# google-research/frame-interpolation

Measured on NVIDIA H100. Metric: interpolated_frames_per_sec_1080p, higher is better.
Workload: dtype f16x2-split (activations/weights as fp16 hi+lo planes; fp32 accumulate)

## Files before the change

### frame_interpolation_b200/csrc/film_conv3x3_tc.cu

```cuda
#include <cuda.h>
#include <cuda_runtime.h>
#include <stdint.h>

#include <type_traits>

#include "film_conv.h"
#include "film_tc_ptx.cuh"

namespace film {
namespace {
using namespace tc;

constexpr int kConsumers = 256;
constexpr int kThreads = kConsumers + 128;
__host__ __device__ constexpr int a_plane_bytes(int kc, int th, int tw) { return (th + 2) * tw * kc * 2; }
__host__ __device__ constexpr int a_stage_bytes(int kc, int th, int tw) { return 2 * a_plane_bytes(kc, th, tw); }
constexpr int kHaloW = 10;
__host__ __device__ constexpr int halo_box_bytes(int kc, int th) { return (th + 2) * kHaloW * kc * 2; }
__host__ __device__ constexpr int halo_plane_bytes(int kc, int th) { return (halo_box_bytes(kc, th) + 1023) & ~1023; }
__host__ __device__ constexpr int a_stage_bytes_h(int kc, int th, int tw, int halo, int planes = 2) {
  return planes * (halo ? halo_plane_bytes(kc, th) : a_plane_bytes(kc, th, tw));
}
constexpr int kMaxRing = 8;
constexpr int kSmemLimit = 227 * 1024;
constexpr int kBarBytes = 8 * (4 * kMaxRing + 4);
constexpr int kFixedBytes = kBarBytes + 16 + 512 * 4  + 64  + 1024  + 64;
constexpr int kHeadW3 = 64 * 32 * 4, kHeadMisc = 512;
constexpr int kHeadBytes = kHeadW3 + kHeadMisc;
constexpr int kPxnStageWg = 64 * 64 * 2;
constexpr int kPxnStageBytes = 2 * kPxnStageWg;
inline int epi_scratch_bytes(int epi_mode, int pxn) { return epi_mode == 3 ? kHeadBytes : pxn ? kPxnStageBytes : 0; }

__host__ __device__ inline int w_tap_bytes(int bn, int kc, int planes = 2) { return bn * kc * 2 * planes; }

template <int BN, int KC, bool kPartial, bool kHalo, bool kOne, bool kRes, bool kPxN = false>
__global__ void __launch_bounds__(kThreads, 1) k_conv3x3_tc(const ConvProblem* __restrict__ prob) {
  static_assert(!kPxN || (BN == 64 && KC == 64), "pixels on N: Cout = 64 (one M = 64 weight tile), 64-channel chunks");
  extern __shared__ uint8_t smem_raw[];
  constexpr bool one = kOne;
  const int planes = one ? 1 : 2;
  constexpr int kWPlane = BN * KC * 2;
  const int kWTap = kWPlane * planes;
  const int kTileH = prob->tile_h, kTileW = prob->tile_w;
  constexpr int kHaloTileH = kPxN ? 32 : 16;
  constexpr int kHaloBox = halo_box_bytes(KC, kHaloTileH), kHaloPlane = halo_plane_bytes(KC, kHaloTileH);
  constexpr bool halo = kHalo;
  const int kAPlane = halo ? kHaloPlane : a_plane_bytes(KC, kTileH, kTileW);
  const int kAStage = planes * kAPlane;
  const int kRowStep = kTileW * KC * 2;
  constexpr bool kFused = BN <= 128 && !kPxN;
  constexpr int kAccRegs = kPxN ? 64 : (kFused ? 2 * BN : BN) / 2;
  constexpr int kWgPx = kPxN ? 128 : 64;

  const int NA = prob->v2_na, NW = prob->v2_nw;
  const bool resident = prob->v2_resident != 0;
  const int nsrc = prob->nsrc;
  const int tiles_x = prob->tiles_x, tiles_per_img = prob->tiles_y * prob->tiles_x;
  const int cout = prob->cout;
  const int n_nt = (cout + BN - 1) / BN;
  const int ntiles = prob->B * tiles_per_img * n_nt;
  constexpr int kStageTaps = kHalo ? 9 : 3;
  constexpr bool kPacked = kPartial && kPxN;
  const int part_lo = prob->v2_part_lo, part_hi = prob->v2_part_hi;
  int nab = 0;
  for (int s = 0; s < nsrc; ++s) nab += prob->src[s].nchunk * (kHalo ? 1 : 3);
  const int nkb = nab * kStageTaps - (kPacked ? (part_hi - part_lo) * (kStageTaps - kStageTaps / 3) : 0);

  const FastDiv div_nt(n_nt, ntiles), div_img(tiles_per_img, ntiles), div_tx(tiles_x, ntiles);
  const bool pair = prob->pair != 0;
  const int rank = pair ? (int)cluster_ctarank() : 0;
  const int nsp = prob->B * tiles_per_img;
  const int nwork = pair ? ((nsp + 1) / 2) * n_nt : ntiles;
  const int w_first = pair ? (int)blockIdx.x >> 1 : (int)blockIdx.x, w_step = pair ? (int)gridDim.x >> 1 : (int)gridDim.x;
  auto decode = [&](int work, int& sp, int& nti) {
    div_nt.divmod(work, sp, nti);
    if (pair) sp = 2 * sp + rank;
  };

  const uint32_t raw = smem_u32(smem_raw);
  const uint32_t base = (raw + 1023u) & ~1023u;
  uint8_t* gen_base = smem_raw + (base - raw);
  const uint32_t a_base = base;
  const uint32_t w_base = a_base + (uint32_t)NA * kAStage;
  const uint32_t w_bytes = resident ? (uint32_t)nkb * kWTap : (uint32_t)NW * kWTap;
  const uint32_t tail = w_base + w_bytes;
  const uint32_t tail_off = (uint32_t)NA * kAStage + w_bytes;
  float* bias_smem = reinterpret_cast<float*>(gen_base + tail_off + kBarBytes + 16);
  int* src_tab = reinterpret_cast<int*>(gen_base + tail_off + kBarBytes + 16 + 512 * 4);

  const int warp = threadIdx.x >> 5, lane = threadIdx.x & 31;

  if (warp == 8 && lane == 0) {
    for (int s = 0; s < kMaxRing; ++s) {
      mbar_init(tail + 8u * s, 1);
      mbar_init(tail + 8u * (kMaxRing + s), 2);
      mbar_init(tail + 8u * (2 * kMaxRing + s), 1);
      mbar_init(tail + 8u * (3 * kMaxRing + s), pair ? 4 : 2);
    }
    for (int s = 0; s < kMaxSrc; ++s) {
      src_tab[2 * s] = s < nsrc ? prob->src[s].nchunk : 0;
      src_tab[2 * s + 1] = s < nsrc ? prob->src[s].c_off : 0;
      src_tab[2 * kMaxSrc + s] = s < nsrc ? prob->src[s].bswap : 0;
    }
    asm volatile("fence.mbarrier_init.release.cluster;" ::: "memory");
  }
  if (warp < 8)
    for (int i = threadIdx.x; i < n_nt * BN; i += kConsumers) bias_smem[i] = (i < cout) ? prob->bias[i] : 0.f;
  __syncthreads();
  if (pair) cluster_sync_all();
  auto leave = [&]() {
    if (pair) cluster_sync_all();
  };

  if (warp >= 8) {
    regs_dec<40>();
    if (warp > 8) {
      leave();
      return;
    }
    const CUtensorMap* tm_w_hi = &prob->tm_w_hi;
    const CUtensorMap* tm_w_lo = &prob->tm_w_lo;
    if (resident && elect_one()) {
      mbar_expect_tx(tail + 8u * (2 * kMaxRing), (uint32_t)nkb * kWTap);
      for (int kb = 0; kb < nkb; ++kb) {
        tma_load_2d(w_base + kb * kWTap, tm_w_hi, tail + 8u * (2 * kMaxRing), kb * KC, 0);
        if (!one) tma_load_2d(w_base + kb * kWTap + kWPlane, tm_w_lo, tail + 8u * (2 * kMaxRing), kb * KC, 0);
      }
    }
    __syncwarp();
    RingPos ra, rw;
    for (int tile = w_first; tile < nwork; tile += w_step) {
      int sp, nti, b, rem, ty, tx;
      decode(tile, sp, nti);
      div_img.divmod(sp, b, rem);
      div_tx.divmod(rem, ty, tx);
      const int n0 = nti * BN, y0 = ty * kTileH, x0 = tx * kTileW;
      {
        const int nt = tile + w_step;
        int next_sp, nnt;
        decode(nt < nwork ? nt : 0, next_sp, nnt);
        if (nt < nwork && next_sp != sp && next_sp < nsp && elect_one()) {
          int nb, nrem, nty, ntx;
          div_img.divmod(next_sp, nb, nrem);
          div_tx.divmod(nrem, nty, ntx);
          const int ny0 = nty * kTileH, nx0 = ntx * kTileW;
          for (int s = 0; s < nsrc; ++s)
            for (int ch = 0; ch < src_tab[2 * s]; ++ch) {
              const int cc = src_tab[2 * s + 1] + ch * KC;
              tma_prefetch_4d(&prob->tm_a_hi[s], cc, nx0 - 1, ny0 - 1, nb);
              if (!one) tma_prefetch_4d(&prob->tm_a_lo[s], cc, nx0 - 1, ny0 - 1, nb);
              if (!halo) {
                tma_prefetch_4d(&prob->tm_a_hi[s], cc, nx0 + 1, ny0 - 1, nb);
                if (!one) tma_prefetch_4d(&prob->tm_a_lo[s], cc, nx0 + 1, ny0 - 1, nb);
              }
            }
        }
        __syncwarp();
      }
      int kb = 0, ab = 0;
      for (int s = 0; s < nsrc; ++s) {
        const int nchunk = src_tab[2 * s], c_off = src_tab[2 * s + 1];
        const int bs = src_tab[2 * kMaxSrc + s] ? prob->B - 1 - b : b;
        const CUtensorMap* tm_hi = &prob->tm_a_hi[s];
        const CUtensorMap* tm_lo = &prob->tm_a_lo[s];
        for (int ch = 0; ch < nchunk; ++ch) {
          const int nst = halo ? 1 : 3;
          for (int dx = 0; dx < nst; ++dx, ++ab) {
            const int st = ra.stage;
            mbar_wait(tail + 8u * (kMaxRing + st), ra.phase ^ 1u);
            if (elect_one()) {
              const uint32_t sa = a_base + st * kAStage, bar = tail + 8u * st;
              mbar_expect_tx(bar, halo ? (uint32_t)(planes * kHaloBox) : (uint32_t)kAStage);
              tma_load_4d(sa, tm_hi, bar, c_off + ch * KC, x0 + dx - 1, y0 - 1, bs);
              if (!one) tma_load_4d(sa + kAPlane, tm_lo, bar, c_off + ch * KC, x0 + dx - 1, y0 - 1, bs);
            }
            __syncwarp();
            ra.advance(NA);
            if (!resident) {
              const bool packed = kPacked && ab >= part_lo && ab < part_hi;
              const int nblk = packed ? kStageTaps / 3 : kStageTaps;
              for (int t = 0; t < nblk; ++t, ++kb) {
                const int ws = rw.stage;
                mbar_wait(tail + 8u * (3 * kMaxRing + ws), rw.phase ^ 1u);
                if (elect_one()) {
                  const uint32_t sw = w_base + ws * kWTap, bar = tail + 8u * (2 * kMaxRing + ws);
                  mbar_expect_tx(bar, kWTap);
                  if (pair) {
                    const uint32_t hoff = (uint32_t)(rank * (kWPlane / 2));
                    tma_load_2d_mc(sw + hoff, &prob->tm_w_hi_half, bar, kb * KC, n0 + rank * (BN / 2), 3);
                    if (!one) tma_load_2d_mc(sw + kWPlane + hoff, &prob->tm_w_lo_half, bar, kb * KC, n0 + rank * (BN / 2), 3);
                  } else {
                    tma_load_2d(sw, tm_w_hi, bar, kb * KC, n0);
                    if (!one) tma_load_2d(sw + kWPlane, tm_w_lo, bar, kb * KC, n0);
                  }
                }
                __syncwarp();
                rw.advance(NW);
              }
            }
          }
        }
      }
    }
    leave();
    return;
  }

  regs_inc<232>();
  const int wg = warp >> 2;
  const int q = lane & 3;
  const int H = prob->H, W = prob->W, out_H = prob->out_H, out_W = prob->out_W, out_C = prob->out_C;
  const int out_c_off = prob->out_c_off, act = prob->act;
  sp_t* const out_hi = prob->out_hi;
  sp_t* const out_lo = prob->out_lo;
  sp_t* const pool_hi = prob->pool_hi;
  sp_t* const pool_lo = prob->pool_lo;
  const int pool_C = prob->pool_C;
  const bool do_pool = pool_hi != nullptr;
  const bool lo_skip = prob->out_lo_skip != 0;
  const bool rgb = prob->epi_mode == 2;
  const float* const head_w = prob->head_w4;
  float* const rgb_out = prob->head_v;
  const int crop_y = prob->crop_y, crop_x = prob->crop_x, crop_h = prob->crop_h, crop_w = prob->crop_w;
  const int64_t crop_pitch = prob->crop_pitch;
  const bool fhead = prob->epi_mode == 3;
  constexpr int kHid = BN <= 64 ? BN / 2 : 1;
  float* const w3s = reinterpret_cast<float*>(reinterpret_cast<uint8_t*>(src_tab) + 64);
  float* const hmisc = w3s + kHeadW3 / 4;
  if (fhead) {
    if constexpr (BN <= 64) {
      for (int i = threadIdx.x; i < BN * kHid; i += kConsumers) w3s[i] = prob->head_w3[i];
      for (int i = threadIdx.x; i < kHid; i += kConsumers) hmisc[i] = prob->head_b3[i];
      for (int i = threadIdx.x; i < 2 * kHid; i += kConsumers) hmisc[kHid + i] = prob->head_w4[i];
      if (threadIdx.x < 2) hmisc[3 * kHid + threadIdx.x] = prob->head_b4[threadIdx.x];
    }
    asm volatile("bar.sync 1, %0;" ::"r"(kConsumers) : "memory");
  }
  const float* const head_vup = prob->head_vup;
  float* const head_res = prob->head_res;
  float* const head_vout = prob->head_v;

  if (resident) mbar_wait(tail + 8u * (2 * kMaxRing), 0);
  const bool is_leader = (threadIdx.x & 127) == 0;
  const uint32_t w_empty_peer = pair ? map_to_cta(tail + 8u * (3 * kMaxRing), (uint32_t)(rank ^ 1)) : 0u;
  auto release_w = [&](int slot) {
    mbar_arrive(tail + 8u * (3 * kMaxRing + slot));
    if (pair) mbar_arrive_cluster(w_empty_peer + 8u * slot);
  };
  {
    constexpr int kWTapC = kWPlane * (kOne ? 1 : 2);
    constexpr uint32_t kPx = KC * 2;
    const uint32_t a_row0 = kHalo ? (uint32_t)(wg * (kWgPx / 8) * kHaloW) * kPx : (uint32_t)(wg * kWgPx) * kPx;
    const uint32_t sbo = kHalo ? kHaloW * kPx : 8 * kPx;
    RingPos ra, rw;
    float acc[kAccRegs];
    for (int tile = w_first; tile < nwork; tile += w_step) {
      int kb = 0;
      int rel_a = -1, rel_w = -1;
      auto retire = [&](int next_a, int next_w) {
        wgmma_commit();
        wgmma_wait<1>();
        if (is_leader) {
          if (rel_a >= 0) mbar_arrive(tail + 8u * (kMaxRing + rel_a));
          if (rel_w >= 0) release_w(rel_w);
        }
        rel_a = next_a;
        rel_w = next_w;
      };
      auto stage = [&](auto ksteps_c, auto tpb_c) {
        constexpr int kSteps = decltype(ksteps_c)::value, kTpb = decltype(tpb_c)::value;
        constexpr int kBlocks = kStageTaps / kTpb;
        const int st = ra.stage;
        mbar_wait(tail + 8u * st, ra.phase);
        const uint32_t sa = a_base + st * kAStage + a_row0;
        const uint32_t lo_off = (uint32_t)(kHalo ? kHaloPlane : kAPlane);
        if constexpr (kRes) {
          const uint64_t a0 = make_desc_sbo<KC>(sa, sbo);
          const uint64_t lo_delta = (uint64_t)(lo_off >> 4);
          const uint64_t row_delta = (uint64_t)(kRowStep >> 4);
          const uint64_t w0 = make_desc_kc<KC>(w_base + kb * kWTapC);
          const uint32_t first = (kb == 0) ? 0u : 1u;
          wgmma_fence();
#pragma unroll
          for (int t = 0; t < kStageTaps; ++t) {
            const uint64_t a_hi = a0 + (kHalo ? (uint64_t)((((t % 3) * kHaloW + t / 3) * kPx) >> 4) : (uint64_t)t * row_delta);
            const uint64_t a_lo = a_hi + lo_delta;
            const uint64_t w_hi = w0 + (uint64_t)(((t / kTpb) * kWTapC + (t % kTpb) * kSteps * 32) >> 4);
            const uint64_t w_lo = w_hi + (uint64_t)(kWPlane >> 4);
#pragma unroll
            for (int k = 0; k < kSteps; ++k) {
              const uint64_t adv = (uint64_t)(k * 32 >> 4);
              const uint32_t accf = (t == 0 && k == 0) ? first : 1u;
              if constexpr (kPxN) {
                wgmma<128>(acc, w_hi + adv, a_hi + adv, accf);
                if constexpr (!kOne) {
                  wgmma<128>(acc, w_lo + adv, a_hi + adv, 1u);
                  wgmma<128>(acc, w_hi + adv, a_lo + adv, 1u);
                }
              } else if constexpr (kOne) {
                wgmma<BN>(acc, a_hi + adv, w_hi + adv, accf);
              } else if constexpr (kFused) {
                wgmma<BN>(acc, a_hi + adv, w_hi + adv, accf);
                wgmma<BN>(acc + BN / 2, a_hi + adv, w_lo + adv, accf);
                wgmma<BN>(acc, a_lo + adv, w_hi + adv, 1u);
              } else {
                wgmma<BN>(acc, a_lo + adv, w_hi + adv, accf);
                wgmma<BN>(acc, a_hi + adv, w_lo + adv, 1u);
                wgmma<BN>(acc, a_hi + adv, w_hi + adv, 1u);
              }
            }
          }
          retire(st, -1);
          kb += kBlocks;
        } else {
          for (int blk = 0; blk < kBlocks; ++blk, ++kb) {
            uint32_t sw;
            int ws = -1;
            if (resident) {
              sw = w_base + kb * kWTap;
            } else {
              ws = rw.stage;
              mbar_wait(tail + 8u * (2 * kMaxRing + ws), rw.phase);
              sw = w_base + ws * kWTap;
            }
            const uint32_t first = (kb == 0) ? 0u : 1u;
            wgmma_fence();
#pragma unroll
            for (int u = 0; u < kTpb; ++u) {
              const int t = blk * kTpb + u;
              const uint32_t off = kHalo ? (uint32_t)((t % 3) * kHaloW + t / 3) * kPx : (uint32_t)(t * kRowStep);
              const uint64_t a_hi = make_desc_sbo<KC>(sa + off, sbo);
              const uint64_t a_lo = make_desc_sbo<KC>(sa + lo_off + off, sbo);
              const uint64_t wk = (uint64_t)((u * kSteps * 32) >> 4);
              const uint64_t w_hi = make_desc_kc<KC>(sw) + wk, w_lo = make_desc_kc<KC>(sw + kWPlane) + wk;
#pragma unroll
              for (int k = 0; k < kSteps; ++k) {
                const uint64_t adv = (uint64_t)(k * 32 >> 4);
                const uint32_t accf = (u == 0 && k == 0) ? first : 1u;
                if constexpr (kPxN) {
                  wgmma<128>(acc, w_hi + adv, a_hi + adv, accf);
                  if constexpr (!kOne) {
                    wgmma<128>(acc, w_lo + adv, a_hi + adv, 1u);
                    wgmma<128>(acc, w_hi + adv, a_lo + adv, 1u);
                  }
                } else if constexpr (kOne) {
                  wgmma<BN>(acc, a_hi + adv, w_hi + adv, accf);
                } else if constexpr (kFused) {
                  wgmma<BN>(acc, a_hi + adv, w_hi + adv, accf);
                  wgmma<BN>(acc + BN / 2, a_hi + adv, w_lo + adv, accf);
                  wgmma<BN>(acc, a_lo + adv, w_hi + adv, 1u);
                } else {
                  wgmma<BN>(acc, a_lo + adv, w_hi + adv, accf);
                  wgmma<BN>(acc, a_hi + adv, w_lo + adv, 1u);
                  wgmma<BN>(acc, a_hi + adv, w_hi + adv, 1u);
                }
              }
            }
            retire(blk == kBlocks - 1 ? st : -1, ws);
            if (!resident) rw.advance(NW);
          }
        }
        ra.advance(NA);
      };
      using Full = std::integral_constant<int, KC / 16>;
      using One = std::integral_constant<int, 1>;
      if constexpr (kPartial) {
        for (int ab = 0; ab < part_lo; ++ab) stage(Full{}, One{});
        for (int ab = part_lo; ab < part_hi; ++ab) stage(One{}, std::integral_constant<int, kPacked ? 3 : 1>{});
        for (int ab = part_hi; ab < nab; ++ab) stage(Full{}, One{});
      } else {
        for (int ab = 0; ab < nab; ++ab) stage(Full{}, One{});
      }
      wgmma_wait<0>();
      if (is_leader) {
        if (rel_a >= 0) mbar_arrive(tail + 8u * (kMaxRing + rel_a));
        if (rel_w >= 0) release_w(rel_w);
      }
      acc_fence<kAccRegs>(acc);

      int sp, nti, b, rem, ty, tx;
      decode(tile, sp, nti);
      div_img.divmod(sp, b, rem);
      div_tx.divmod(rem, ty, tx);
      const int n0 = nti * BN;
      const bool live = sp < nsp;
      if constexpr (kPxN) {
        const int c0 = 16 * (warp & 3) + (lane >> 2);
        const float bias0 = bias_smem[c0], bias1 = bias_smem[c0 + 8];
#pragma unroll
        for (int i = 0; i < kAccRegs; ++i) {
          const float f = acc[i] + ((i & 2) ? bias1 : bias0);
          acc[i] = act ? leaky(f) : f;
        }
        const int y_wg = ty * kTileH + 16 * wg, x_t = tx * kTileW;
        if (do_pool) {
          const int px = x_t + 2 * q;
#pragma unroll
          for (int j = 0; j < 16; j += 2) {
            const int py = y_wg + j;
            const bool ok = live && (py >> 1) < (out_H >> 1) && (px >> 1) < (out_W >> 1) && !(lane & 4);
            const int64_t ppix = ((int64_t)b * (out_H >> 1) + (py >> 1)) * (out_W >> 1) + (px >> 1);
#pragma unroll
            for (int h = 0; h < 2; ++h) {
              const int i = 4 * j + 2 * h;
              const float v = ((acc[i] + acc[i + 1]) + (acc[i + 4] + acc[i + 5])) * 0.25f;
              const float vn = __shfl_xor_sync(0xffffffffu, v, 4);
              if (ok) {
                uint32_t hi, lo;
                split_pack2(v, vn, hi, lo);
                *reinterpret_cast<uint32_t*>(pool_hi + ppix * pool_C + c0 + 8 * h) = hi;
                *reinterpret_cast<uint32_t*>(pool_lo + ppix * pool_C + c0 + 8 * h) = lo;
              }
            }
          }
        }
        uint8_t* const stg = reinterpret_cast<uint8_t*>(src_tab) + 64 + wg * kPxnStageWg;
        const uint32_t stg_u = smem_u32(stg);
        const int t128 = threadIdx.x & 127;
        auto wg_sync = [&]() { asm volatile("bar.sync %0, 128;" ::"r"(2 + wg) : "memory"); };
        for (int pl = 0; pl < (lo_skip ? 1 : 2); ++pl) {
          sp_t* const dst = pl ? out_lo : out_hi;
#pragma unroll
          for (int half = 0; half < 2; ++half) {
            wg_sync();
#pragma unroll
            for (int jj = 0; jj < 8; jj += 2) {
              uint32_t r[4];
#pragma unroll
              for (int m = 0; m < 4; ++m) {
                const int i = 4 * (8 * half + jj + (m >> 1)) + 2 * (m & 1);
                if (pl) {
                  uint32_t hi;
                  split_pack2(acc[i], acc[i + 1], hi, r[m]);
                } else {
                  r[m] = pack2_hi(acc[i], acc[i + 1]);
                }
              }
              const int p = 8 * (jj + (lane >> 4)) + (lane & 7), ch = 2 * (warp & 3) + ((lane >> 3) & 1);
              stmatrix_x4_trans(stg_u + p * 128 + ((ch ^ (p & 7)) << 4), r[0], r[1], r[2], r[3]);
            }
            wg_sync();
#pragma unroll
            for (int k = 0; k < 4; ++k) {
              const int idx = 128 * k + t128, p = idx >> 3, ch = idx & 7;
              const int py = y_wg + 8 * half + (p >> 3), px = x_t + (p & 7);
              if (live && py < H && px < W) {
                const uint4 v = *reinterpret_cast<const uint4*>(stg + p * 128 + ((ch ^ (p & 7)) << 4));
                const int64_t opix = ((int64_t)b * out_H + py) * out_W + px;
                *reinterpret_cast<uint4*>(dst + opix * out_C + out_c_off + 8 * ch) = v;
              }
            }
          }
        }
        continue;
      }
      auto value = [&](int h, int j, int e) {
        const int i = 4 * j + 2 * h + e;
        return (kFused && !kOne) ? acc[i] + acc[(i + BN / 2) % kAccRegs] : acc[i];
      };
#pragma unroll
      for (int h = 0; h < 2 && (fhead || rgb); ++h) {
        const int r = wg * 64 + (warp & 3) * 16 + (lane >> 2) + 8 * h;
        const int py = ty * kTileH + r / kTileW, px = tx * kTileW + r % kTileW;
        const bool valid = live && (py < H) && (px < W);
        const int64_t opix = ((int64_t)b * out_H + py) * out_W + px;
        if (fhead) {
          if constexpr (BN <= 64) {
            float hp[kHid];
#pragma unroll
            for (int hh = 0; hh < kHid; ++hh) hp[hh] = 0.f;
#pragma unroll
            for (int j = 0; j < BN / 8; ++j)
#pragma unroll
              for (int e = 0; e < 2; ++e) {
                const int c = 8 * j + 2 * q + e;
                const float x = value(h, j, e) + bias_smem[n0 + c];
                const float f = act ? leaky(x) : x;
                const float4* wr = reinterpret_cast<const float4*>(w3s + c * kHid);
#pragma unroll
                for (int h4 = 0; h4 < kHid / 4; ++h4) {
                  const float4 wv = wr[h4];
                  hp[4 * h4] = fmaf(f, wv.x, hp[4 * h4]);
                  hp[4 * h4 + 1] = fmaf(f, wv.y, hp[4 * h4 + 1]);
                  hp[4 * h4 + 2] = fmaf(f, wv.z, hp[4 * h4 + 2]);
                  hp[4 * h4 + 3] = fmaf(f, wv.w, hp[4 * h4 + 3]);
                }
              }
#pragma unroll
            for (int hh = 0; hh < kHid; ++hh) {
              hp[hh] += __shfl_xor_sync(0xffffffffu, hp[hh], 1);
              hp[hh] += __shfl_xor_sync(0xffffffffu, hp[hh], 2);
            }
            if (q == 0 && valid) {
              float f0 = hmisc[3 * kHid], f1 = hmisc[3 * kHid + 1];
#pragma unroll
              for (int hh = 0; hh < kHid; ++hh) {
                const float x = leaky(hp[hh] + hmisc[hh]);
                f0 = fmaf(x, hmisc[kHid + 2 * hh], f0);
                f1 = fmaf(x, hmisc[kHid + 2 * hh + 1], f1);
              }
              float2 res = make_float2(f0, f1), tot = res;
              if (head_vup) {
                const float2 u = reinterpret_cast<const float2*>(head_vup)[opix];
                tot.x += u.x;
                tot.y += u.y;
              }
              reinterpret_cast<float2*>(head_res)[opix] = res;
              reinterpret_cast<float2*>(head_vout)[opix] = tot;
            }
          }
        } else if (rgb) {
          float r0 = 0.f, r1 = 0.f, r2 = 0.f;
#pragma unroll
          for (int j = 0; j < BN / 8; ++j)
#pragma unroll
            for (int e = 0; e < 2; ++e) {
              const int c = n0 + 8 * j + 2 * q + e;
              float f = value(h, j, e) + bias_smem[c];
              if (act) f = leaky(f);
              r0 = fmaf(f, __ldg(head_w + 3 * c), r0);
              r1 = fmaf(f, __ldg(head_w + 3 * c + 1), r1);
              r2 = fmaf(f, __ldg(head_w + 3 * c + 2), r2);
            }
#pragma unroll
          for (int m = 1; m <= 2; m <<= 1) {
            r0 += __shfl_xor_sync(0xffffffffu, r0, m);
            r1 += __shfl_xor_sync(0xffffffffu, r1, m);
            r2 += __shfl_xor_sync(0xffffffffu, r2, m);
          }
          const int oy = py - crop_y, ox = px - crop_x;
          if (q == 0 && valid && oy >= 0 && oy < crop_h && ox >= 0 && ox < crop_w) {
            float* o = rgb_out + (int64_t)oy * crop_pitch + (int64_t)ox * 3;
            o[0] = r0 + __ldg(prob->head_b4);
            o[1] = r1 + __ldg(prob->head_b4 + 1);
            o[2] = r2 + __ldg(prob->head_b4 + 2);
          }
        }
      }
      if (!fhead && !rgb) {
        bool valid[2];
        int64_t opix[2];
#pragma unroll
        for (int h = 0; h < 2; ++h) {
          const int r = wg * 64 + (warp & 3) * 16 + (lane >> 2) + 8 * h;
          const int py = ty * kTileH + r / kTileW, px = tx * kTileW + r % kTileW;
          valid[h] = live && (py < H) && (px < W);
          opix[h] = ((int64_t)b * out_H + py) * out_W + px;
        }
        const int r0 = wg * 64 + (warp & 3) * 16 + (lane >> 2);
        const int py0 = ty * kTileH + r0 / kTileW, px0 = tx * kTileW + r0 % kTileW;
        const bool pool_ok = live && (py0 >> 1) < (out_H >> 1) && (px0 >> 1) < (out_W >> 1) && !(lane & 4);
        const int64_t ppix = ((int64_t)b * (out_H >> 1) + (py0 >> 1)) * (out_W >> 1) + (px0 >> 1);
#pragma unroll
        for (int j = 0; j < BN / 8; ++j) {
          const int c = 8 * j + 2 * q;
          if (n0 + c >= cout) break;
          float a[2][2];
#pragma unroll
          for (int h = 0; h < 2; ++h) {
            float f0 = value(h, j, 0) + bias_smem[n0 + c], f1 = value(h, j, 1) + bias_smem[n0 + c + 1];
            if (act) {
              f0 = leaky(f0);
              f1 = leaky(f1);
            }
            if (valid[h]) {
              sp_t* oh = out_hi + opix[h] * out_C + out_c_off + n0;
              if (lo_skip) {
                *reinterpret_cast<uint32_t*>(oh + c) = pack2_hi(f0, f1);
              } else {
                sp_t* ol = out_lo + opix[h] * out_C + out_c_off + n0;
                uint32_t hi, lo;
                split_pack2(f0, f1, hi, lo);
                *reinterpret_cast<uint32_t*>(oh + c) = hi;
                *reinterpret_cast<uint32_t*>(ol + c) = lo;
              }
            }
            if (do_pool) {
              a[h][0] = f0 + __shfl_xor_sync(0xffffffffu, f0, 4);
              a[h][1] = f1 + __shfl_xor_sync(0xffffffffu, f1, 4);
            }
          }
          if (do_pool && pool_ok) {
            uint32_t hi, lo;
            split_pack2((a[0][0] + a[1][0]) * 0.25f, (a[0][1] + a[1][1]) * 0.25f, hi, lo);
            *reinterpret_cast<uint32_t*>(pool_hi + ppix * pool_C + n0 + c) = hi;
            *reinterpret_cast<uint32_t*>(pool_lo + ppix * pool_C + n0 + c) = lo;
          }
        }
      }
    }
  }
  leave();
}

int smem_bytes_for(const ConvProblem& h, int bn) {
  const int nkb = h.ktot / h.kchunk;
  const int planes = h.passes == 1 ? 1 : 2;
  const int w = h.v2_resident ? nkb * w_tap_bytes(bn, h.kchunk, planes) : h.v2_nw * w_tap_bytes(bn, h.kchunk, planes);
  return h.v2_na * a_stage_bytes_h(h.kchunk, h.tile_h, h.tile_w, h.halo, planes) + w + kFixedBytes +
         epi_scratch_bytes(h.epi_mode, h.pxn);
}

}

int conv_tc_block_n(int cout);

namespace {
bool ring_depths(int kc, int tile_h, int tile_w, int halo, int planes, int bn, int cout, int ktot, int epi_mode, int pxn,
                 int& resident, int& na, int& nw) {
  const int wtap = w_tap_bytes(bn, kc, planes);
  const int w_all = (ktot / kc) * wtap;
  const int kLimit = kSmemLimit - epi_scratch_bytes(epi_mode, pxn);
  const int kAStage = a_stage_bytes_h(kc, tile_h, tile_w, halo, planes);
  if (cout <= bn && w_all + 2 * kAStage + kFixedBytes <= kLimit) {
    resident = 1;
    const int n = (kLimit - kFixedBytes - w_all) / kAStage;
    const int n_max = halo ? 3 : 6;
    na = n > n_max ? n_max : n;
    nw = 1;
    return true;
  }
  resident = 0;
  na = halo ? 2 : (bn >= 128 ? 2 : 3);
  int n = (kLimit - kFixedBytes - na * kAStage) / wtap;
  if (n < 2 && na > 2) {
    na = 2;
    n = (kLimit - kFixedBytes - na * kAStage) / wtap;
  }
  nw = n > kMaxRing ? kMaxRing : n;
  return nw >= 2;
}
}

void conv3x3_tc_pick_tile(int H, int W, int B, int cout, int kc, int passes, int ktot, int epi_mode, int num_sms,
                          int& tile_h, int& tile_w) {
  static const int cand[3][2] = {{16, 8}, {8, 16}, {4, 32}};
  const int bn = conv_tc_block_n(cout);
  const int n_nt = (cout + bn - 1) / bn;
  double best = 1e30;
  tile_h = 16;
  tile_w = 8;
  for (auto& c : cand) {
    int res, na, nw;
    if (!ring_depths(kc, c[0], c[1], 0, passes == 1 ? 1 : 2, bn, cout, ktot, epi_mode, 0, res, na, nw)) continue;
    const long tiles = (long)B * ((H + c[0] - 1) / c[0]) * ((W + c[1] - 1) / c[1]) * n_nt;
    const long waves = (tiles + num_sms - 1) / num_sms;
    const double cost = (double)waves * (c[0] + 2.0) / c[0] * (1.0 + 1e-3 * (c[1] / 8));
    if (cost < best) {
      best = cost;
      tile_h = c[0];
      tile_w = c[1];
    }
  }
}

bool conv3x3_tc_plan(ConvProblem& h, int num_sms) {
  const int bn = h.bn;
  const int planes = h.passes == 1 ? 1 : 2;
  const int wtap = w_tap_bytes(bn, h.kchunk, planes);
  const int w_all = (h.ktot / h.kchunk) * wtap;
  const bool can_resident = h.cout <= bn;
  const int kLimit = kSmemLimit - epi_scratch_bytes(h.epi_mode, h.pxn);
  if (h.halo && (h.tile_h != (h.pxn ? 32 : 16) || h.tile_w != 8 ||
                 (can_resident && w_all + 2 * a_stage_bytes_h(h.kchunk, h.tile_h, h.tile_w, 0, planes) + kFixedBytes <= kLimit &&
                  w_all + 2 * a_stage_bytes_h(h.kchunk, h.tile_h, h.tile_w, 1, planes) + kFixedBytes > kLimit)))
    h.halo = 0;
  bool ok = ring_depths(h.kchunk, h.tile_h, h.tile_w, h.halo, planes, bn, h.cout, h.ktot, h.epi_mode, h.pxn,
                        h.v2_resident, h.v2_na, h.v2_nw);
  if (!ok && h.halo) {
    h.halo = 0;
    ok = ring_depths(h.kchunk, h.tile_h, h.tile_w, 0, planes, bn, h.cout, h.ktot, h.epi_mode, h.pxn, h.v2_resident,
                     h.v2_na, h.v2_nw);
  }
  const int nsp = h.B * h.tiles_y * h.tiles_x, n_nt = (h.cout + bn - 1) / bn;
  if (h.pair) {
    const int nwork = (nsp + 1) / 2 * n_nt, nclu = num_sms / 2;
    h.v2_grid = 2 * (nwork < nclu ? nwork : nclu);
  } else {
    h.v2_grid = nsp * n_nt < num_sms ? nsp * n_nt : num_sms;
  }
  return ok;
}

template <int BN, int KC, bool kPxN = false>
struct Variants {
  static constexpr void (*kFn[16])(const ConvProblem*) = {
      k_conv3x3_tc<BN, KC, false, false, false, false, kPxN>, k_conv3x3_tc<BN, KC, false, false, false, true, kPxN>,
      k_conv3x3_tc<BN, KC, false, false, true, false, kPxN>,  k_conv3x3_tc<BN, KC, false, false, true, true, kPxN>,
      k_conv3x3_tc<BN, KC, false, true, false, false, kPxN>,  k_conv3x3_tc<BN, KC, false, true, false, true, kPxN>,
      k_conv3x3_tc<BN, KC, false, true, true, false, kPxN>,   k_conv3x3_tc<BN, KC, false, true, true, true, kPxN>,
      k_conv3x3_tc<BN, KC, true, false, false, false, kPxN>,  k_conv3x3_tc<BN, KC, true, false, false, true, kPxN>,
      k_conv3x3_tc<BN, KC, true, false, true, false, kPxN>,   k_conv3x3_tc<BN, KC, true, false, true, true, kPxN>,
      k_conv3x3_tc<BN, KC, true, true, false, false, kPxN>,   k_conv3x3_tc<BN, KC, true, true, false, true, kPxN>,
      k_conv3x3_tc<BN, KC, true, true, true, false, kPxN>,    k_conv3x3_tc<BN, KC, true, true, true, true, kPxN>};
  static cudaError_t configure() {
    for (auto fn : kFn) {
      const cudaError_t e = cudaFuncSetAttribute(fn, cudaFuncAttributeMaxDynamicSharedMemorySize, kSmemLimit);
      if (e != cudaSuccess) return e;
    }
    return cudaSuccess;
  }
  static cudaError_t launch(const ConvProblem* d_prob, const ConvProblem& h, cudaStream_t st) {
    if (h.v2_na < 2 || (!h.v2_resident && h.v2_nw < 2)) return cudaErrorInvalidValue;
    if (kPxN && (h.pair || h.tile_h != 32 || h.tile_w != 8 || h.epi_mode != 0)) return cudaErrorInvalidValue;
    const bool partial = h.v2_part_hi > h.v2_part_lo;
    const int idx = (partial ? 8 : 0) | (h.halo ? 4 : 0) | (h.passes == 1 ? 2 : 0) | (h.v2_resident && h.straight ? 1 : 0);
    if (!h.pair) {
      kFn[idx]<<<h.v2_grid, kThreads, smem_bytes_for(h, BN), st>>>(d_prob);
      return cudaGetLastError();
    }
    cudaLaunchConfig_t cfg = {};
    cudaLaunchAttribute attr[1];
    attr[0].id = cudaLaunchAttributeClusterDimension;
    attr[0].val.clusterDim.x = 2;
    attr[0].val.clusterDim.y = 1;
    attr[0].val.clusterDim.z = 1;
    cfg.gridDim = dim3(h.v2_grid);
    cfg.blockDim = dim3(kThreads);
    cfg.dynamicSmemBytes = smem_bytes_for(h, BN);
    cfg.stream = st;
    cfg.attrs = attr;
    cfg.numAttrs = 1;
    return cudaLaunchKernelEx(&cfg, kFn[idx], d_prob);
  }
};

cudaError_t conv3x3_tc_configure() {
  cudaError_t e;
#define FILM_CFG(BN, KC)                        \
  e = Variants<BN, KC>::configure();            \
  if (e != cudaSuccess) return e;
  FILM_CFG(32, 64) FILM_CFG(64, 64) FILM_CFG(128, 64) FILM_CFG(256, 64) FILM_CFG(32, 32) FILM_CFG(64, 32)
#undef FILM_CFG
  e = Variants<64, 64, true>::configure();
  if (e != cudaSuccess) return e;
  return cudaSuccess;
}

cudaError_t launch_conv3x3_tc(const ConvProblem* d_prob, const ConvProblem& h, cudaStream_t st) {
  const int bn = h.bn;
  if (h.kchunk == 32) {
    if (bn == 32) return Variants<32, 32>::launch(d_prob, h, st);
    if (bn == 64) return Variants<64, 32>::launch(d_prob, h, st);
    return cudaErrorInvalidValue;
  }
  switch (bn) {
    case 256: return Variants<256, 64>::launch(d_prob, h, st);
    case 128: return Variants<128, 64>::launch(d_prob, h, st);
    case 64: return h.pxn ? Variants<64, 64, true>::launch(d_prob, h, st) : Variants<64, 64>::launch(d_prob, h, st);
    default: return Variants<32, 64>::launch(d_prob, h, st);
  }
}

}
```

### frame_interpolation_b200/csrc/film_engine.cu

```cuda
#include <cuda.h>
#include <cuda_runtime.h>

#include <algorithm>
#include <cmath>
#include <cstdio>
#include <cstdlib>
#include <cstring>
#include <functional>
#include <map>
#include <memory>
#include <string>
#include <vector>

#include "../../include/film_b200.h"
#include "film_conv.h"
#include "film_kernels.h"
#include "film_pack.h"

namespace film {
int conv_tc_block_n(int cout);

constexpr int kLevels = 7, kFusionLevels = 5, kSpecialized = 3, kSubLevels = 4, kFilters = 64;
static const int kFlowFilters[4] = {32, 64, 128, 256};
static const char* kPredictorNames[4] = {"flow_predictor_0", "flow_predictor_1", "flow_predictor_2",
// ... 453 lines not shown
};
struct SrcRef {
  const SplitBuf* buf;
  int c_off;
  int bswap;
};
struct DebugTensor {
  bool split;
  const void* p0;
  const void* p1;
  int64_t npix;
  int C, c_off, Cn;
  bool recycled = false;
};

struct Plan {
  int h, w, H, W, off_y, off_x;
  Options opt;
  int num_sms = 132;
  bool onepass(int stage) const { return stage >= 0 && opt.conv_impl == 0 && (((uint32_t)opt.onepass_mask >> stage) & 1u); }
  bool hi_only(int consumer) const { return opt.plane_skip && onepass(consumer); }
  std::vector<void*> allocs;
  int64_t arena_bytes = 0;
  std::vector<ConvProblem> h_probs;
  ConvProblem* d_probs = nullptr;
  struct Op {
    std::function<cudaError_t(cudaStream_t)> fn;
    int category;
    std::string name;
    double flops;
    double bytes;
    int lane;
    std::vector<int> waits;
    std::vector<int> signals;
    std::string form = "";
    int passes = 0;
  };
  std::vector<Op> ops;
  std::vector<float> op_ms;
  static constexpr int kNumLanes = 8;
  int cur_lane = 0, num_tokens = 0, tok_end = -1;
  std::vector<int> pending_waits;
  int new_token() { return num_tokens++; }
  void add_op(int category, const std::string& name, std::function<cudaError_t(cudaStream_t)> fn,
              double flops = 0, double bytes = 0) {
    ops.push_back(Op{std::move(fn), category, name, flops, bytes, cur_lane, pending_waits, {}});
    pending_waits.clear();
  }
  void signal_last(int token) { ops.back().signals.push_back(token); }
  std::map<std::string, DebugTensor> debug;
  float* xin = nullptr;
  float* xout = nullptr;
  float* time = nullptr;
  cudaGraphExec_t graph = nullptr;
  double conv_flops = 0, mma_flops = 0, warp_bytes = 0, last_conv_bytes = 0;
  bool times = false;
  size_t tail_begin = 0;
  int tok_head = -1;
  cudaGraphExec_t graph_tail = nullptr;
  double head_conv_flops = 0, head_mma_flops = 0, head_warp_bytes = 0;

  bool reuse = true;
  std::map<void*, int64_t> block_bytes;
  std::multimap<int64_t, void*> free_blocks;
  template <class T>
  T* alloc(int64_t count, bool pinned = false) {
    const int64_t bytes = std::max<int64_t>(count * (int64_t)sizeof(T), 256);
    if (reuse && !pinned) {
      auto it = free_blocks.lower_bound(bytes);
      if (it != free_blocks.end() && it->first <= 2 * bytes) {
        void* p = it->second;
        free_blocks.erase(it);
        return (T*)p;
      }
    }
    void* p;
    FILM_CUDA(cudaMalloc(&p, bytes));
    allocs.push_back(p);
    FILM_CUDA(cudaMemset(p, 0, bytes));
    arena_bytes += bytes;
    if (!pinned) block_bytes[p] = bytes;
    return (T*)p;
  }
  void release(void* p) {
    if (!reuse || !p) return;
    auto it = block_bytes.find(p);
    if (it != block_bytes.end()) free_blocks.insert({it->second, p});
  }
  void release(const SplitBuf* s) {
    if (!s) return;
    release((void*)s->hi);
    release((void*)s->lo);
  }
  SplitBuf* split(int B, int H_, int W_, int C, bool pinned = false) {
    bufs.emplace_back(new SplitBuf);
    SplitBuf* s = bufs.back().get();
    s->B = B;
    s->H = H_;
    s->W = W_;
    s->C = C;
    s->hi = alloc<sp_t>((int64_t)B * H_ * W_ * C, pinned);
    s->lo = alloc<sp_t>((int64_t)B * H_ * W_ * C, pinned);
    return s;
  }
  std::vector<std::unique_ptr<SplitBuf>> bufs;

  ~Plan() {
    if (graph) cudaGraphExecDestroy(graph);
    if (graph_tail) cudaGraphExecDestroy(graph_tail);
    for (void* p : allocs) cudaFree(p);
  }
};

static void pick_tile(int H, int W, int& th, int& tw) {
  static const int cand[][2] = {{8, 16}, {16, 8}, {4, 32}, {32, 4}, {2, 64}, {64, 2}, {1, 128}, {128, 1}};
  long best = -1;
  for (auto& c : cand) {
    long tiles = (long)((H + c[0] - 1) / c[0]) * ((W + c[1] - 1) / c[1]);
    if (best < 0 || tiles < best) {
      best = tiles;
      th = c[0];
      tw = c[1];
    }
  }
}

static size_t add_conv(Plan& P, const std::string& tag, double ref_macs_per_px, const PackedConv& pc,
                       const std::vector<SrcRef>& sources, int act, const SplitBuf* out, int out_c_off,
                       int stage, int consumer, int sy = 1, int sx = 1, int oy = 0, int ox = 0,
                       const SplitBuf* pool_out = nullptr, bool no_op = false, int epi_mode = 0) {
  const Options& o = P.opt;
  ConvProblem cp;
  memset(&cp, 0, sizeof(cp));
  cp.passes = P.onepass(stage) ? 1 : 3;
  cp.out_lo_skip = (!pool_out && P.hi_only(consumer)) ? 1 : 0;
  cp.straight = o.mma_straight;
  const SplitBuf* s0 = sources[0].buf;
  cp.nsrc = (int)sources.size();
  if (cp.nsrc != (int)pc.src_chunks.size()) throw Error{FILM_ERR_WEIGHTS, "source count mismatch"};
  cp.B = s0->B;
  cp.H = s0->H;
  cp.W = s0->W;
  const int kc = pc.kchunk;
  cp.kchunk = kc;
  const bool v2 = o.conv3x3_v2 && o.conv_impl == 0 && pc.ntaps == 9 && (out || epi_mode >= 2) && sy == 1 && sx == 1 &&
                  (kc == kChunk || pc.cout <= 64);
  cp.epi_mode = epi_mode;
  const auto waves = [&](long tiles) { return (tiles + P.num_sms - 1) / P.num_sms; };
  const long pxn_tiles = (long)cp.B * ((cp.H + 31) / 32) * ((cp.W + 7) / 8);
  const long tiles16 = (long)cp.B * ((cp.H + 15) / 16) * ((cp.W + 7) / 8);
  bool skips_ksteps = false;
  for (size_t s = 0; s < pc.src_chunks.size(); ++s)
    if (pc.src_chunks[s] > 0 && pc.src_ksteps[s] != kc / 16) skips_ksteps = true;
  const bool pxn_pays = skips_ksteps ? 2 * waves(pxn_tiles) <= waves(tiles16) : pxn_tiles >= 2L * P.num_sms;
  cp.pxn = (v2 && o.conv3x3_pxn && pc.cout == 64 && kc == kChunk && epi_mode == 0 && out && out_c_off % 8 == 0 &&
            out->C % 8 == 0 && (!pool_out || pool_out->C % 8 == 0) && (o.conv3x3_pxn >= 2 || pxn_pays)) ? 1 : 0;
  const int ktot = cp.pxn ? pc.pxn_ktot : pc.ktot;
  const sp_t* w_hi = cp.pxn ? pc.pxn_hi : pc.w_hi;
  const sp_t* w_lo = cp.pxn ? pc.pxn_lo : pc.w_lo;
  int box_h, box_w;
  if (v2) {
    if (cp.pxn) {
      cp.tile_h = 32;
      cp.tile_w = 8;
    } else if (pool_out) {
      cp.tile_h = 16;
      cp.tile_w = 8;
    } else {
      conv3x3_tc_pick_tile(cp.H, cp.W, cp.B, pc.cout, kc, cp.passes, ktot, epi_mode, P.num_sms, cp.tile_h, cp.tile_w);
    }
    box_h = cp.tile_h + 2;
    box_w = cp.tile_w;
  } else {
    pick_tile(cp.H, cp.W, cp.tile_h, cp.tile_w);
    box_h = cp.tile_h;
    box_w = cp.tile_w;
  }
  cp.tiles_y = (cp.H + cp.tile_h - 1) / cp.tile_h;
  cp.tiles_x = (cp.W + cp.tile_w - 1) / cp.tile_w;
  for (int s = 0; s < cp.nsrc; ++s) {
    const SplitBuf* b = sources[s].buf;
    if (b->B != cp.B || b->H != cp.H || b->W != cp.W) throw Error{FILM_ERR_ARG, "conv source grid mismatch"};
    cp.src[s].hi = b->hi;
    cp.src[s].lo = b->lo;
    cp.src[s].C = b->C;
    cp.src[s].c_off = sources[s].c_off;
    cp.src[s].nchunk = pc.src_chunks[s];
    cp.src[s].bswap = sources[s].bswap;
    if (sources[s].c_off + pc.src_chunks[s] * kc > b->C) throw Error{FILM_ERR_ARG, "conv source channel overrun"};
    make_act_map(&cp.tm_a_hi[s], b->hi, b->B, b->H, b->W, b->C, box_h, box_w, kc);
    make_act_map(&cp.tm_a_lo[s], b->lo, b->B, b->H, b->W, b->C, box_h, box_w, kc);
  }
  cp.ntaps = pc.ntaps;
  for (int t = 0; t < pc.ntaps; ++t) {
    cp.tap_dy[t] = pc.tap_dy[t];
    cp.tap_dx[t] = pc.tap_dx[t];
  }
  cp.ktot = ktot;
  cp.w_hi = w_hi;
  cp.w_lo = w_lo;
  cp.bias = pc.bias;
  cp.cout = pc.cout;
  cp.act = act;
  int bn = conv_tc_block_n(pc.cout);
  if (out && !pool_out) {
    auto items = [&](int b) { return (long)cp.B * cp.tiles_y * cp.tiles_x * ((pc.cout + b - 1) / b); };
    while (bn > 64 && 2 * items(bn) <= P.num_sms) bn /= 2;
  }
  cp.bn = bn;
  make_w_map(&cp.tm_w_hi, w_hi, pc.cout, ktot, bn, kc);
  make_w_map(&cp.tm_w_lo, w_lo, pc.cout, ktot, bn, kc);
  make_w_map(&cp.tm_w_hi_half, w_hi, pc.cout, ktot, bn / 2, kc);
  make_w_map(&cp.tm_w_lo_half, w_lo, pc.cout, ktot, bn / 2, kc);
  if (out) {
    cp.out_hi = out->hi;
    cp.out_lo = out->lo;
    cp.out_C = out->C;
    cp.out_H = out->H;
    cp.out_W = out->W;
  } else {
    cp.out_C = 0;
    cp.out_H = cp.H;
    cp.out_W = cp.W;
  }
  cp.out_c_off = out_c_off;
  cp.out_sy = sy;
  cp.out_sx = sx;
  cp.out_oy = oy;
  cp.out_ox = ox;
  if (out && (out->B != cp.B || out_c_off + pc.cout > out->C)) throw Error{FILM_ERR_ARG, "conv destination mismatch"};
  if (pool_out) {
    if (!v2) throw Error{FILM_ERR_UNSUPPORTED, "fused pool needs the persistent 3x3 kernel"};
    cp.pool_hi = pool_out->hi;
    cp.pool_lo = pool_out->lo;
    cp.pool_C = pool_out->C;
  }
  cp.group = 1;
  int halo_ok = (v2 && cp.tile_h == (cp.pxn ? 32 : 16) && cp.tile_w == 8) ? o.conv3x3_halo : 0;
  if (kc != kChunk && halo_ok < 3) halo_ok = 0;
  if (cp.pxn && skips_ksteps) halo_ok = 0;
  cp.halo = halo_ok >= 2;
  if (v2 && !conv3x3_tc_plan(cp, P.num_sms))
    throw Error{FILM_ERR_UNSUPPORTED, "persistent 3x3 conv: shared-memory rings do not fit (" + tag + ")"};
  if (v2 && o.conv3x3_2cta && epi_mode < 2 && !cp.v2_resident && !cp.pxn &&
      (o.conv3x3_2cta >= 2 || (long)cp.B * cp.tiles_y * cp.tiles_x >= 4L * P.num_sms)) {
    cp.pair = 1;
    if (halo_ok >= 1) cp.halo = 1;
    if (!conv3x3_tc_plan(cp, P.num_sms))
      throw Error{FILM_ERR_UNSUPPORTED, "persistent 3x3 conv: shared-memory rings do not fit (" + tag + ")"};
  }
  if (cp.halo) {
    for (int s = 0; s < cp.nsrc; ++s) {
      const SplitBuf* b = sources[s].buf;
      make_act_map(&cp.tm_a_hi[s], b->hi, b->B, b->H, b->W, b->C, box_h, box_w + 2, kc);
      make_act_map(&cp.tm_a_lo[s], b->lo, b->B, b->H, b->W, b->C, box_h, box_w + 2, kc);
    }
  }
  if (v2) {
    const int nst = cp.halo ? 1 : 3;
    for (int s = 0, ab = 0; s < cp.nsrc; ab += pc.src_chunks[s] * nst, ++s) {
      if (pc.src_chunks[s] == 0 || pc.src_ksteps[s] == kc / 16) continue;
      if (pc.src_ksteps[s] != 1 || cp.v2_part_hi > cp.v2_part_lo)
        throw Error{FILM_ERR_UNSUPPORTED, "persistent 3x3 conv: only one source may skip k-steps, and it must issue one (" +
                                              tag + ")"};
      cp.v2_part_lo = ab;
      cp.v2_part_hi = ab + pc.src_chunks[s] * nst;
    }
  }
  const size_t idx = P.h_probs.size();
  P.h_probs.push_back(cp);
  double k_issued = 0;
  for (size_t si = 0; si < pc.src_chunks.size(); ++si)
    k_issued += (double)pc.src_chunks[si] * pc.ntaps * (v2 ? pc.src_ksteps[si] * 16 : pc.kchunk);
  P.mma_flops += (double)cp.passes * 2.0 * (double)cp.B * cp.tiles_y * cp.tiles_x * (cp.tile_h * cp.tile_w) * k_issued *
                 (double)(((pc.cout + bn - 1) / bn) * bn);
  double alg_bytes = 0;
  {
    const double px = (double)cp.B * cp.H * cp.W, planes_in = cp.passes == 1 ? 1.0 : 2.0;
    for (size_t si = 0; si < pc.src_chunks.size(); ++si) alg_bytes += px * pc.src_chunks[si] * pc.kchunk * 2.0 * planes_in;
    if (out) alg_bytes += px * pc.cout * 2.0 * (cp.out_lo_skip ? 1.0 : 2.0);
    if (pool_out) alg_bytes += px / 4.0 * pc.cout * 4.0;
    if (epi_mode == 2) alg_bytes += px * 12.0;
    if (!out && epi_mode != 2) alg_bytes += px * 24.0;
    alg_bytes += (double)pc.cout * ktot * 2.0 * planes_in;
  }
  P.last_conv_bytes = alg_bytes;
  if (out && sy == 1 && sx == 1 && !tag.empty())
    P.debug["out:" + tag] = DebugTensor{true, out->hi, out->lo, out->pixels(), out->C, out_c_off, pc.cout};
  if (pool_out)
    P.debug["pool:" + tag] = DebugTensor{true, pool_out->hi, pool_out->lo, pool_out->pixels(), pool_out->C, 0, pc.cout};
  if (no_op) return idx;
  Plan* pp = &P;
  const int impl = o.conv_impl;
  P.add_op(0, tag, [pp, idx, impl, v2](cudaStream_t st) {
    if (impl == 1) return launch_conv_simt(pp->d_probs + idx, pp->h_probs[idx], st);
    return v2 ? launch_conv3x3_tc(pp->d_probs + idx, pp->h_probs[idx], st)
              : launch_conv_tc(pp->d_probs + idx, pp->h_probs[idx], st);
  }, 2.0 * ref_macs_per_px * (double)cp.B * cp.H * cp.W, alg_bytes);
  P.ops.back().form = impl == 1 ? "simt" : !v2 ? "tc" : cp.pxn ? "3x3_pxn" : cp.pair ? "3x3_pair" : "3x3";
  P.ops.back().passes = cp.passes;
  return idx;
}

static void padded_size(int h, int w, int align, int& H, int& W, int& off_y, int& off_x) {
  int ph = 0, pw = 0;
  if (align > 0) {
    ph = (h % align) ? align - h % align : 0;
    pw = (w % align) ? align - w % align : 0;
  }
  H = h + ph;
  W = w + pw;
  off_y = ph / 2;
  off_x = pw / 2;
}

static std::unique_ptr<Plan> build_plan(const Model& M, int h, int w, int align, const Options& opt, int num_sms,
                                        bool times) {
  std::unique_ptr<Plan> pl(new Plan);
  Plan& P = *pl;
  P.opt = opt;
  P.times = times;
  P.reuse = !opt.keep_debug && !opt.use_lanes && opt.arena_reuse;
  const bool fuse_rgb = opt.conv_impl == 0 && opt.conv3x3_v2 && opt.fuse_rgb_head;
  P.h = h;
  P.w = w;
  P.num_sms = num_sms;
  padded_size(h, w, align, P.H, P.W, P.off_y, P.off_x);
  int Hs[kLevels], Ws[kLevels];
  for (int l = 0; l < kLevels; ++l) {
    Hs[l] = P.H >> l;
    Ws[l] = P.W >> l;
  }
  if (Hs[kLevels - 2] < 2 || Ws[kLevels - 2] < 2) throw Error{FILM_ERR_ARG, "frame too small"};

  P.xin = P.alloc<float>((int64_t)2 * h * w * 3, true);
  P.xout = P.alloc<float>((int64_t)h * w * 3, true);
  {
    const float half = 0.5f;
    FILM_CUDA(cudaMalloc(&P.time, sizeof(float)));
    P.allocs.push_back(P.time);
    FILM_CUDA(cudaMemcpy(P.time, &half, sizeof(float), cudaMemcpyHostToDevice));
  }
  Plan* pp = &P;

  float* img[kLevels];
  for (int l = 0; l < kLevels; ++l) {
    img[l] = P.alloc<float>((int64_t)2 * Hs[l] * Ws[l] * 3, true);
    P.debug["img/" + std::to_string(l)] = DebugTensor{false, img[l], nullptr, (int64_t)2 * Hs[l] * Ws[l], 3, 0, 3};
  }
  for (int k = 0; k < 2; ++k) {
    float* dst = img[0] + (int64_t)k * P.H * P.W * 3;
    const float* src = P.xin + (int64_t)k * h * w * 3;
    P.add_op(2, "pad_image", [=](cudaStream_t st) {
      return launch_pad_image(src, (int64_t)pp->w * 3, pp->h, pp->w, dst, pp->H, pp->W, pp->off_y, pp->off_x, st);
    });
  }
  const bool fuse_img_pool = opt.conv_impl == 0 && !opt.fe_conv0_tc && !opt.use_lanes;
// ... 1373 lines not shown
```

Baseline: 26.41.

## Extend pixels-on-N conv3x3 path to wider Cout with two M tiles

Generalizes the pixels-on-N wgmma conv3x3 kernel from Cout=64 to BN=128 by issuing two M=64 weight tiles per k-step into a doubled accumulator, and extends the bias/pool/store epilogue over both halves with an n0 channel offset. The engine now enables this path for Cout 128/256/512 layers when single-pass and not skipping k-steps, capping BN at 128 and gating on a work-count heuristic. The intent is to raise tensor-core efficiency on wider layers, at the cost of doubled accumulator registers and extra tile items for 256/512 channels.

```diff
diff --git a/frame_interpolation_b200/csrc/film_conv3x3_tc.cu b/frame_interpolation_b200/csrc/film_conv3x3_tc.cu
--- a/frame_interpolation_b200/csrc/film_conv3x3_tc.cu
+++ b/frame_interpolation_b200/csrc/film_conv3x3_tc.cu
@@ -35,7 +35,7 @@
 
 template <int BN, int KC, bool kPartial, bool kHalo, bool kOne, bool kRes, bool kPxN = false>
 __global__ void __launch_bounds__(kThreads, 1) k_conv3x3_tc(const ConvProblem* __restrict__ prob) {
-  static_assert(!kPxN || (BN == 64 && KC == 64), "pixels on N: Cout = 64 (one M = 64 weight tile), 64-channel chunks");
+  static_assert(!kPxN || ((BN == 64 || BN == 128) && KC == 64), "pixels on N: one or two M = 64 weight tiles, 64-channel chunks");
   extern __shared__ uint8_t smem_raw[];
   constexpr bool one = kOne;
   const int planes = one ? 1 : 2;
@@ -49,7 +49,8 @@
   const int kAStage = planes * kAPlane;
   const int kRowStep = kTileW * KC * 2;
   constexpr bool kFused = BN <= 128 && !kPxN;
-  constexpr int kAccRegs = kPxN ? 64 : (kFused ? 2 * BN : BN) / 2;
+  constexpr int kMh = kPxN ? BN / 64 : 1;
+  constexpr int kAccRegs = kPxN ? 64 * kMh : (kFused ? 2 * BN : BN) / 2;
   constexpr int kWgPx = kPxN ? 128 : 64;
 
   const int NA = prob->v2_na, NW = prob->v2_nw;
@@ -254,6 +255,17 @@
     const uint32_t sbo = kHalo ? kHaloW * kPx : 8 * kPx;
     RingPos ra, rw;
     float acc[kAccRegs];
+    auto pxn_mma = [&](uint64_t w_hi, uint64_t w_lo, uint64_t a_hi, uint64_t a_lo, uint32_t accf) {
+#pragma unroll
+      for (int h = 0; h < kMh; ++h) {
+        const uint64_t wh = (uint64_t)(h * (64 * KC * 2) >> 4);
+        wgmma<128>(acc + 64 * h, w_hi + wh, a_hi, accf);
+        if constexpr (!kOne) {
+          wgmma<128>(acc + 64 * h, w_lo + wh, a_hi, 1u);
+          wgmma<128>(acc + 64 * h, w_hi + wh, a_lo, 1u);
+        }
+      }
+    };
     for (int tile = w_first; tile < nwork; tile += w_step) {
       int kb = 0;
       int rel_a = -1, rel_w = -1;
@@ -292,11 +304,7 @@
               const uint64_t adv = (uint64_t)(k * 32 >> 4);
               const uint32_t accf = (t == 0 && k == 0) ? first : 1u;
               if constexpr (kPxN) {
-                wgmma<128>(acc, w_hi + adv, a_hi + adv, accf);
-                if constexpr (!kOne) {
-                  wgmma<128>(acc, w_lo + adv, a_hi + adv, 1u);
-                  wgmma<128>(acc, w_hi + adv, a_lo + adv, 1u);
-                }
+                pxn_mma(w_hi + adv, w_lo + adv, a_hi + adv, a_lo + adv, accf);
               } else if constexpr (kOne) {
                 wgmma<BN>(acc, a_hi + adv, w_hi + adv, accf);
               } else if constexpr (kFused) {
@@ -338,11 +346,7 @@
                 const uint64_t adv = (uint64_t)(k * 32 >> 4);
                 const uint32_t accf = (u == 0 && k == 0) ? first : 1u;
                 if constexpr (kPxN) {
-                  wgmma<128>(acc, w_hi + adv, a_hi + adv, accf);
-                  if constexpr (!kOne) {
-                    wgmma<128>(acc, w_lo + adv, a_hi + adv, 1u);
-                    wgmma<128>(acc, w_hi + adv, a_lo + adv, 1u);
-                  }
+                  pxn_mma(w_hi + adv, w_lo + adv, a_hi + adv, a_lo + adv, accf);
                 } else if constexpr (kOne) {
                   wgmma<BN>(acc, a_hi + adv, w_hi + adv, accf);
                 } else if constexpr (kFused) {
@@ -386,11 +390,14 @@
       const bool live = sp < nsp;
       if constexpr (kPxN) {
         const int c0 = 16 * (warp & 3) + (lane >> 2);
-        const float bias0 = bias_smem[c0], bias1 = bias_smem[c0 + 8];
-#pragma unroll
-        for (int i = 0; i < kAccRegs; ++i) {
-          const float f = acc[i] + ((i & 2) ? bias1 : bias0);
-          acc[i] = act ? leaky(f) : f;
+#pragma unroll
+        for (int m = 0; m < kMh; ++m) {
+          const float bias0 = bias_smem[n0 + 64 * m + c0], bias1 = bias_smem[n0 + 64 * m + c0 + 8];
+#pragma unroll
+          for (int i = 64 * m; i < 64 * m + 64; ++i) {
+            const float f = acc[i] + ((i & 2) ? bias1 : bias0);
+            acc[i] = act ? leaky(f) : f;
+          }
         }
         const int y_wg = ty * kTileH + 16 * wg, x_t = tx * kTileW;
         if (do_pool) {
@@ -401,17 +408,20 @@
             const bool ok = live && (py >> 1) < (out_H >> 1) && (px >> 1) < (out_W >> 1) && !(lane & 4);
             const int64_t ppix = ((int64_t)b * (out_H >> 1) + (py >> 1)) * (out_W >> 1) + (px >> 1);
 #pragma unroll
-            for (int h = 0; h < 2; ++h) {
-              const int i = 4 * j + 2 * h;
-              const float v = ((acc[i] + acc[i + 1]) + (acc[i + 4] + acc[i + 5])) * 0.25f;
-              const float vn = __shfl_xor_sync(0xffffffffu, v, 4);
-              if (ok) {
-                uint32_t hi, lo;
-                split_pack2(v, vn, hi, lo);
-                *reinterpret_cast<uint32_t*>(pool_hi + ppix * pool_C + c0 + 8 * h) = hi;
-                *reinterpret_cast<uint32_t*>(pool_lo + ppix * pool_C + c0 + 8 * h) = lo;
-              }
-            }
+            for (int m = 0; m < kMh; ++m)
+#pragma unroll
+              for (int h = 0; h < 2; ++h) {
+                const int i = 64 * m + 4 * j + 2 * h;
+                const float v = ((acc[i] + acc[i + 1]) + (acc[i + 4] + acc[i + 5])) * 0.25f;
+                const float vn = __shfl_xor_sync(0xffffffffu, v, 4);
+                if (ok) {
+                  uint32_t hi, lo;
+                  split_pack2(v, vn, hi, lo);
+                  const int64_t pc = ppix * pool_C + n0 + 64 * m + c0 + 8 * h;
+                  *reinterpret_cast<uint32_t*>(pool_hi + pc) = hi;
+                  *reinterpret_cast<uint32_t*>(pool_lo + pc) = lo;
+                }
+              }
           }
         }
         uint8_t* const stg = reinterpret_cast<uint8_t*>(src_tab) + 64 + wg * kPxnStageWg;
@@ -419,38 +429,40 @@
         const int t128 = threadIdx.x & 127;
         auto wg_sync = [&]() { asm volatile("bar.sync %0, 128;" ::"r"(2 + wg) : "memory"); };
         for (int pl = 0; pl < (lo_skip ? 1 : 2); ++pl) {
-          sp_t* const dst = pl ? out_lo : out_hi;
-#pragma unroll
-          for (int half = 0; half < 2; ++half) {
-            wg_sync();
-#pragma unroll
-            for (int jj = 0; jj < 8; jj += 2) {
-              uint32_t r[4];
-#pragma unroll
-              for (int m = 0; m < 4; ++m) {
-                const int i = 4 * (8 * half + jj + (m >> 1)) + 2 * (m & 1);
-                if (pl) {
-                  uint32_t hi;
-                  split_pack2(acc[i], acc[i + 1], hi, r[m]);
-                } else {
-                  r[m] = pack2_hi(acc[i], acc[i + 1]);
+          sp_t* const dst = (pl ? out_lo : out_hi) + out_c_off + n0;
+#pragma unroll
+          for (int m = 0; m < kMh; ++m)
+#pragma unroll
+            for (int half = 0; half < 2; ++half) {
+              wg_sync();
+#pragma unroll
+              for (int jj = 0; jj < 8; jj += 2) {
+                uint32_t r[4];
+#pragma unroll
+                for (int mm = 0; mm < 4; ++mm) {
+                  const int i = 64 * m + 4 * (8 * half + jj + (mm >> 1)) + 2 * (mm & 1);
+                  if (pl) {
+                    uint32_t hi;
+                    split_pack2(acc[i], acc[i + 1], hi, r[mm]);
+                  } else {
+                    r[mm] = pack2_hi(acc[i], acc[i + 1]);
+                  }
                 }
-              }
-              const int p = 8 * (jj + (lane >> 4)) + (lane & 7), ch = 2 * (warp & 3) + ((lane >> 3) & 1);
-              stmatrix_x4_trans(stg_u + p * 128 + ((ch ^ (p & 7)) << 4), r[0], r[1], r[2], r[3]);
-            }
-            wg_sync();
-#pragma unroll
-            for (int k = 0; k < 4; ++k) {
-              const int idx = 128 * k + t128, p = idx >> 3, ch = idx & 7;
-              const int py = y_wg + 8 * half + (p >> 3), px = x_t + (p & 7);
-              if (live && py < H && px < W) {
-                const uint4 v = *reinterpret_cast<const uint4*>(stg + p * 128 + ((ch ^ (p & 7)) << 4));
-                const int64_t opix = ((int64_t)b * out_H + py) * out_W + px;
-                *reinterpret_cast<uint4*>(dst + opix * out_C + out_c_off + 8 * ch) = v;
-              }
-            }
-          }
+                const int p = 8 * (jj + (lane >> 4)) + (lane & 7), ch = 2 * (warp & 3) + ((lane >> 3) & 1);
+                stmatrix_x4_trans(stg_u + p * 128 + ((ch ^ (p & 7)) << 4), r[0], r[1], r[2], r[3]);
+              }
+              wg_sync();
+#pragma unroll
+              for (int k = 0; k < 4; ++k) {
+                const int idx = 128 * k + t128, p = idx >> 3, ch = idx & 7;
+                const int py = y_wg + 8 * half + (p >> 3), px = x_t + (p & 7);
+                if (live && py < H && px < W) {
+                  const uint4 v = *reinterpret_cast<const uint4*>(stg + p * 128 + ((ch ^ (p & 7)) << 4));
+                  const int64_t opix = ((int64_t)b * out_H + py) * out_W + px;
+                  *reinterpret_cast<uint4*>(dst + opix * out_C + 64 * m + 8 * ch) = v;
+                }
+              }
+            }
         }
         continue;
       }
@@ -734,6 +746,8 @@
 #undef FILM_CFG
   e = Variants<64, 64, true>::configure();
   if (e != cudaSuccess) return e;
+  e = Variants<128, 64, true>::configure();
+  if (e != cudaSuccess) return e;
   return cudaSuccess;
 }
 
@@ -746,7 +760,7 @@
   }
   switch (bn) {
     case 256: return Variants<256, 64>::launch(d_prob, h, st);
-    case 128: return Variants<128, 64>::launch(d_prob, h, st);
+    case 128: return h.pxn ? Variants<128, 64, true>::launch(d_prob, h, st) : Variants<128, 64>::launch(d_prob, h, st);
     case 64: return h.pxn ? Variants<64, 64, true>::launch(d_prob, h, st) : Variants<64, 64>::launch(d_prob, h, st);
     default: return Variants<32, 64>::launch(d_prob, h, st);
   }
diff --git a/frame_interpolation_b200/csrc/film_engine.cu b/frame_interpolation_b200/csrc/film_engine.cu
--- a/frame_interpolation_b200/csrc/film_engine.cu
+++ b/frame_interpolation_b200/csrc/film_engine.cu
@@ -629,9 +629,14 @@
   bool skips_ksteps = false;
   for (size_t s = 0; s < pc.src_chunks.size(); ++s)
     if (pc.src_chunks[s] > 0 && pc.src_ksteps[s] != kc / 16) skips_ksteps = true;
-  const bool pxn_pays = skips_ksteps ? 2 * waves(pxn_tiles) <= waves(tiles16) : pxn_tiles >= 2L * P.num_sms;
-  cp.pxn = (v2 && o.conv3x3_pxn && pc.cout == 64 && kc == kChunk && epi_mode == 0 && out && out_c_off % 8 == 0 &&
-            out->C % 8 == 0 && (!pool_out || pool_out->C % 8 == 0) && (o.conv3x3_pxn >= 2 || pxn_pays)) ? 1 : 0;
+  const bool wide = (pc.cout == 128 || pc.cout == 256 || pc.cout == 512) && cp.passes == 1 && !skips_ksteps;
+  const bool wide_pays = pc.cout == 128 || (pc.cout == 256 && pc.ktot <= 9 * 1024);
+  const long pxn_items = pxn_tiles * (wide ? pc.cout / 128 : 1);
+  const bool pxn_pays = skips_ksteps ? 2 * waves(pxn_tiles) <= waves(tiles16)
+                                     : pxn_items >= 2L * P.num_sms && (pc.cout == 64 || wide_pays);
+  cp.pxn = (v2 && o.conv3x3_pxn && (pc.cout == 64 || wide) && kc == kChunk && epi_mode == 0 && out &&
+            out_c_off % 8 == 0 && out->C % 8 == 0 && (!pool_out || pool_out->C % 8 == 0) &&
+            (o.conv3x3_pxn >= 2 || pxn_pays)) ? 1 : 0;
   const int ktot = cp.pxn ? pc.pxn_ktot : pc.ktot;
   const sp_t* w_hi = cp.pxn ? pc.pxn_hi : pc.w_hi;
   const sp_t* w_lo = cp.pxn ? pc.pxn_lo : pc.w_lo;
@@ -680,6 +685,7 @@
   cp.cout = pc.cout;
   cp.act = act;
   int bn = conv_tc_block_n(pc.cout);
+  if (cp.pxn && bn > 128) bn = 128;
   if (out && !pool_out) {
     auto items = [&](int b) { return (long)cp.B * cp.tiles_y * cp.tiles_x * ((pc.cout + b - 1) / b); };
     while (bn > 64 && 2 * items(bn) <= P.num_sms) bn /= 2;
```

After: 27.23, median of 6. +3.1%, better.
